# sczhou/CodeFormer

Measured on NVIDIA H100. Metric: faces_per_sec_512x512_batch32, higher is better.
Workload: dtype f32 (split-fp16 operands on tensor cores, fp32 accumulate)

## Files before the change

### codeformer_b200/csrc/conv_tc.cu

```cuda

#include <cuda.h>
#include <cuda_fp16.h>
#include <cuda_runtime.h>
#include <stdint.h>

#include <stdlib.h>

#include <atomic>
#include <mutex>

#include "conv_tc.cuh"

namespace cfb {

__global__ void tc_absmax_kernel(const float* __restrict__ w, int64_t total, unsigned* __restrict__ slot) {
  float m = 0.f;
  for (int64_t i = (int64_t)blockIdx.x * blockDim.x + threadIdx.x; i < total; i += (int64_t)gridDim.x * blockDim.x)
    m = fmaxf(m, fabsf(w[i]));
#pragma unroll
  for (int o = 16; o > 0; o >>= 1) m = fmaxf(m, __shfl_xor_sync(0xffffffffu, m, o));
  if ((threadIdx.x & 31) == 0) atomicMax(slot, __float_as_uint(m));
}

__global__ void tc_split_weights_kernel(const float* __restrict__ w, __half* __restrict__ hi, __half* __restrict__ lo,
// ... 445 lines not shown
  int a_split;
  const float* in_scale;
  const float* in_shift;
  int in_act;
  const float* bias;
  const float* residual;
  int out_act;
  const float* sft_dec;
  const float* sft_scale;
  union {
    float sft_w;
    float prelu;
  };
  const float* wscale_inv;
  float* out;
  __half* pl_hi;
  __half* pl_lo;
  float* gn_part;
  int gn_cpg;
  const float* sft_wv;
#if CFB_TC_STAMPS
  long long* dbg;
#endif
};
#if CFB_TC_STAMPS
#define TC_STAMP(i) do { if (p.dbg != nullptr && blockIdx.x == 0) p.dbg[i] = clock64(); } while (0)
#else
#define TC_STAMP(i) do { } while (0)
#endif

constexpr int XF_SKEW = 128;
constexpr int TC_A_BYTES = 128 * 128;

template <int BN>
struct TcCfg {
  static_assert(BN == 64 || BN == 128, "the wgmma engine runs 64- or 128-wide n-tiles");
  static constexpr bool WIDE = BN == 128;
  static constexpr int MMA_WARPS = WIDE ? 8 : 4;
  static constexpr int EPI_WARPS = WIDE ? 4 : 8;
  static constexpr int THREADS = WIDE ? 512 : 32 * (MMA_WARPS + 1 + EPI_WARPS);
  static constexpr int B_BYTES = BN * 128;
  static constexpr int STAGE_BYTES = 2 * TC_A_BYTES + 2 * B_BYTES;
  static constexpr int STAGES = 3;
  static constexpr int SLOT_PITCH = BN + 4;
  static constexpr int SLOT_BYTES = 128 * SLOT_PITCH * 4;
  static constexpr int SLOTS = 1;
  static constexpr int STG_BYTES = WIDE ? 0 : 8 * 4096;
  static constexpr int TAIL_BYTES = SLOT_BYTES + 1024  + 512  + STG_BYTES;
  static constexpr int SMEM_BYTES = STAGES * STAGE_BYTES + TAIL_BYTES;
  static constexpr int H_A_PLANE = 23 * 1024;
  static constexpr int H_A_SLOT = 2 * H_A_PLANE;
  static constexpr int H_A_SLOTS = 2;
  static constexpr int H_B_SLOT = 2 * B_BYTES;
  static constexpr int H_B_SLOTS = WIDE ? 2 : 4;
  static constexpr int H_SMEM_BYTES = H_A_SLOTS * H_A_SLOT + H_B_SLOTS * H_B_SLOT + TAIL_BYTES;
  static constexpr int XF_WARPS = WIDE ? 2 : 4;
  static constexpr int XF_THREADS = 32 * (MMA_WARPS + 1 + EPI_WARPS + XF_WARPS + 1);
  static_assert(!WIDE || XF_THREADS == THREADS, "the 128-wide transform variant fills the pad warps exactly");
  static constexpr int X_A_SLOTS = 2;
  static constexpr int X_A_PLANE2 = H_A_PLANE + XF_SKEW;
  static constexpr int X_B_SLOTS = H_B_SLOTS;
  static constexpr int X_SMEM_BYTES = X_A_SLOTS * H_A_SLOT + X_B_SLOTS * H_B_SLOT + TAIL_BYTES;
};

template <int BN, int CPG, bool HALO, bool XF, bool GEN = false, bool K1 = false, bool CM = false, bool SILU = false,
          bool P1 = false, bool PRELU = false>
__global__ void __launch_bounds__(XF ? TcCfg<BN>::XF_THREADS : TcCfg<BN>::THREADS, 1)
conv_tc_kernel(const __grid_constant__ CUtensorMap tmA_hi, const __grid_constant__ CUtensorMap tmA_lo,
               const __grid_constant__ CUtensorMap tmB_hi, const __grid_constant__ CUtensorMap tmB_lo, const TcParams p) {
  static_assert(!XF || HALO, "the fused operand transform exists for the halo engine only");
  static_assert(!GEN || (XF && CPG == 0), "the generalised addressing exists for the fused-transform engine only");
  static_assert(!PRELU || (BN == 64 && CPG == 0 && !K1 && !CM && !SILU && !P1 && (GEN || !HALO)),
                "the PReLU epilogue is built for the generalised and the per-tap engines");
  static_assert(!K1 || (XF && !GEN && CPG == 0), "K1 = fused transform of a 1x1 conv (patch = tile): its own instantiation");
  using Cfg = TcCfg<BN>;
  constexpr bool WIDE = Cfg::WIDE;
  static_assert(!WIDE || (HALO && !GEN && !K1 && CPG != 2), "128-wide tiles exist for the 3x3 / Upsample halo engine");
  static_assert(!CM || (BN == 64 && HALO && !GEN && !K1), "channel-major tiles exist for the 64-channel 3x3 / Upsample halo convs");
  static_assert(!P1 || (!SILU && !K1 && (GEN || WIDE || CM || !HALO)),
                "the single-pass fp16 variant is built for the generalised, 128-wide, channel-major and per-tap engines");
  constexpr int MMA_WARPS = Cfg::MMA_WARPS, EPI_WARPS = Cfg::EPI_WARPS;
  constexpr int A_SLOTS = XF ? Cfg::X_A_SLOTS : Cfg::H_A_SLOTS;
  constexpr int STAGES = Cfg::STAGES;
  constexpr int STAGE_BYTES = Cfg::STAGE_BYTES;
  const int first_tile = (int)blockIdx.x;
  const int tile_step = (int)gridDim.x;
  extern __shared__ uint8_t smem_raw[];
  uint8_t* smem = reinterpret_cast<uint8_t*>((reinterpret_cast<uintptr_t>(smem_raw) + 1023) & ~(uintptr_t)1023);
  constexpr int NRING = HALO ? (XF ? Cfg::X_B_SLOTS : Cfg::H_B_SLOTS) : STAGES;
  constexpr int RING_BYTES = HALO ? Cfg::H_B_SLOT : STAGE_BYTES;
  uint8_t* ring_base = HALO ? smem + A_SLOTS * Cfg::H_A_SLOT : smem;
  float* acc_slot = reinterpret_cast<float*>(ring_base + NRING * RING_BYTES);
  uint64_t* bars = reinterpret_cast<uint64_t*>(ring_base + NRING * RING_BYTES + Cfg::SLOT_BYTES);
  uint64_t* full = bars;
  uint64_t* empty = bars + NRING;
  uint64_t* cfull = bars + 2 * NRING;
  uint64_t* cempty = bars + 2 * NRING + Cfg::SLOTS;
  uint64_t* afull = bars + 2 * NRING + 2 * Cfg::SLOTS;
  uint64_t* aempty = afull + 3;
  uint64_t* araw = aempty + 3;
  uint8_t* stage_buf = reinterpret_cast<uint8_t*>(bars) + 512;

  constexpr int NWARPS = (XF ? Cfg::XF_THREADS : Cfg::THREADS) / 32;
  const int pwarp = __shfl_sync(0xffffffffu, (int)(threadIdx.x >> 5), 0);
  const int ridx = NWARPS - 1 - pwarp;
  const int warp = pwarp < MMA_WARPS ? 1 : (ridx == 0 ? 0 : ridx + 1);
  const int lane = threadIdx.x & 31;
  bool aborted = false;
  if constexpr (WIDE) {
    if (pwarp >= MMA_WARPS) wg_regs_dec<96>();
  }
  if (threadIdx.x == 0) TC_STAMP(0);

  if (warp == 0 && lane == 0) {
    for (int a = 0; a < 3; ++a) {
      mbar_init(smem_u32(afull + a), XF ? Cfg::XF_WARPS : 1);
      mbar_init(smem_u32(aempty + a), MMA_WARPS);
      mbar_init(smem_u32(araw + a), 1);
    }
    asm volatile("prefetch.tensormap [%0];" ::"l"(&tmA_hi) : "memory");
    asm volatile("prefetch.tensormap [%0];" ::"l"(&tmA_lo) : "memory");
    asm volatile("prefetch.tensormap [%0];" ::"l"(&tmB_hi) : "memory");
    asm volatile("prefetch.tensormap [%0];" ::"l"(&tmB_lo) : "memory");
    for (int s = 0; s < NRING; ++s) { mbar_init(smem_u32(full + s), 1); mbar_init(smem_u32(empty + s), MMA_WARPS); }
    for (int a = 0; a < Cfg::SLOTS; ++a) {
      mbar_init(smem_u32(cfull + a), MMA_WARPS);
      mbar_init(smem_u32(cempty + a), EPI_WARPS);
    }
    asm volatile("fence.mbarrier_init.release.cluster;" ::: "memory");
  }
  __syncthreads();
  pdl_launch_dependents();
  pdl_wait();
  if (threadIdx.x == 0) TC_STAMP(1);

  const int total_tiles = p.m_tiles * p.n_tiles;
  const int nk = p.taps * p.kblocks;

  if (warp == 0) {
    {
      int stage = 0;
      uint32_t phase = 0;
      int aslot = 0;
// ... 38 lines not shown
            }
          }
        } else {
          for (int tap = 0; tap < p.taps; ++tap) {
            int r, s, btap = tap;
            if (p.up4) { r = (tap >> 1) + par_y; s = (tap & 1) + par_x; btap = (mt & 3) * 4 + tap; }
            else { r = (p.taps == 9) ? tap / 3 : 0; s = (p.taps == 9) ? tap - r * 3 : 0; }
            for (int kb = 0; kb < p.kblocks; ++kb) {
              mbar_wait<500>(smem_u32(empty + stage), phase ^ 1, aborted); if (aborted) goto teardown;
              if (elect_one()) {
                if (tile == first_tile && tap == 0 && kb == 0) TC_STAMP(2);
                const uint32_t sa = smem_u32(smem + stage * STAGE_BYTES);
                const int hh = p.heads > 1 ? n % p.heads : 0, nimg = p.heads > 1 ? n / p.heads : n;
                const int a_img = p.a_img_per_head ? n : nimg;
                const int ac = p.a_c0 + hh * p.a_c_head + kb * 64, bc = p.b_c0 + hh * p.b_c_head + kb * 64;
                const int brow = nt * BN + hh * p.b_r_head;
                const int b3 = p.b_batched ? nimg : btap;
                const uint32_t fb = smem_u32(full + stage);
                const bool drop = p.fault && blockIdx.x == 0 && tile == first_tile && kb == 0 && tap == 0;
                mbar_expect_tx(fb, (uint32_t)(P1 ? TC_A_BYTES + Cfg::B_BYTES : Cfg::STAGE_BYTES));
                tma_load_4d(sa, &tmA_hi, fb, ac, x0 + s - p.pad, y0 + r - p.pad, a_img);
                if constexpr (!P1) tma_load_4d(sa + TC_A_BYTES, &tmA_lo, fb, ac, x0 + s - p.pad, y0 + r - p.pad, a_img);
                if (!drop) tma_load_3d(sa + 2 * TC_A_BYTES, &tmB_hi, fb, bc, brow, b3);
                if constexpr (!P1) tma_load_3d(sa + 2 * TC_A_BYTES + Cfg::B_BYTES, &tmB_lo, fb, bc, brow, b3);
              }
              __syncwarp();
              if (++stage == STAGES) { stage = 0; phase ^= 1; }
            }
          }
        }
      }
    }
  } else if (warp == 1) {
    if constexpr (WIDE) wg_regs_inc<160>();
    {
      constexpr bool N128 = WIDE || CM;
      constexpr int MH = N128 ? 1 : 2;
      const uint32_t a_sbo = HALO ? (uint32_t)(p.PW * 128) : 1024u;
      const uint32_t a_half = HALO ? (uint32_t)(8 * p.PW * 128) : 8192u;
      const int wq = (int)(threadIdx.x >> 5) & 3;
      const int wg = (int)(threadIdx.x >> 7);
      const uint32_t bar_id = 2u + (uint32_t)wg;
      const uint32_t slot_base = smem_u32(acc_slot);
      int stage = 0;
      uint32_t phase = 0;
      int slot = 0;
      uint32_t slot_phase = 0;
      int aslot = 0;
      uint32_t aphase = 0;
      float acc[MH][N128 ? 64 : 32];
      if constexpr (N128) {
        float run[64];
        auto hand_off = [&]() -> bool {
          mbar_wait(smem_u32(cempty + slot), slot_phase ^ 1, aborted);
          if (wg_any(aborted, bar_id)) return true;
          const int row = wg * 64 + wq * 16 + (lane >> 2);
          uint32_t e0;
          asm volatile("mov.b32 %0, %1;" : "=r"(e0)
                       : "r"(slot_base + (uint32_t)(slot * Cfg::SLOT_BYTES) + (uint32_t)((row * Cfg::SLOT_PITCH + 2 * (lane & 3)) * 4)));
#pragma unroll
          for (int j = 0; j < 16; ++j) {
#pragma unroll
            for (int h8 = 0; h8 < 2; ++h8) {
              const uint32_t e = e0 + (uint32_t)((8 * h8 * Cfg::SLOT_PITCH + 8 * j) * 4);
              asm volatile("st.shared.v2.f32 [%0], {%1, %2};" ::"r"(e), "f"(run[4 * j + 2 * h8]), "f"(run[4 * j + 2 * h8 + 1])
                           : "memory");
            }
          }
          __syncwarp();
          if (lane == 0) mbar_arrive(smem_u32(cfull + slot));
          if (++slot == Cfg::SLOTS) { slot = 0; slot_phase ^= 1; }
          return false;
        };
        for (int tile = first_tile; tile < total_tiles; tile += tile_step) {
          const int par = p.up4 ? ((tile / p.n_tiles) & 3) : 0;
          const int par_y = par >> 1, par_x = par & 1;
          for (int c0 = 0; c0 < nk; c0 += p.chunk) {
            const int c1 = min(c0 + p.chunk, nk);
            uint32_t prev_empty = 0, prev_aempty = 0;
            for (int it = c0; it < c1; ++it) {
              const int kb = it / p.taps;
              const int tap = it - kb * p.taps;
              if (tap == 0) {
                mbar_wait(smem_u32(afull + aslot), aphase, aborted);
                if (wg_any(aborted, bar_id)) { wg_wait_all(); aborted = true; goto teardown; }
              }
              int r = (p.taps == 9) ? tap / 3 : 0;
              int sft = (p.taps == 9) ? tap - r * 3 : 0;
              if (p.up4) { r = (tap >> 1) + par_y; sft = (tap & 1) + par_x; }
              const uint32_t a_hi0 = smem_u32(smem + aslot * Cfg::H_A_SLOT) + (uint32_t)((r * p.PW + sft) * 128) +
                                     (uint32_t)wg * a_half;
              const uint32_t a_lo0 = a_hi0 + (uint32_t)(XF ? Cfg::X_A_PLANE2 : Cfg::H_A_PLANE);
              const uint32_t bsm = smem_u32(ring_base + stage * RING_BYTES);
              mbar_wait(smem_u32(full + stage), phase, aborted);
              if (wg_any(aborted, bar_id)) { wg_wait_all(); aborted = true; goto teardown; }
              wg_fence();
#pragma unroll
              for (int k = 0; k < 4; ++k) {
                const uint64_t db_hi = wg_desc(bsm + 32 * k, 1024u), db_lo = wg_desc(bsm + Cfg::B_BYTES + 32 * k, 1024u);
                const uint64_t da_hi = wg_desc(a_hi0 + 32 * k, a_sbo), da_lo = wg_desc(a_lo0 + 32 * k, a_sbo);
                if constexpr (P1 && CM) {
                  wg_mma_64x128(acc[0], db_hi, da_hi, (it == c0 && k == 0) ? 0u : 1u);
                } else if constexpr (P1) {
                  wg_mma_64x128(acc[0], da_hi, db_hi, (it == c0 && k == 0) ? 0u : 1u);
                } else if constexpr (CM) {
                  wg_mma_64x128(acc[0], db_hi, da_lo, (it == c0 && k == 0) ? 0u : 1u);
                  wg_mma_64x128(acc[0], db_lo, da_hi, 1u);
                  wg_mma_64x128(acc[0], db_hi, da_hi, 1u);
                } else {
                  wg_mma_64x128(acc[0], da_lo, db_hi, (it == c0 && k == 0) ? 0u : 1u);
                  wg_mma_64x128(acc[0], da_hi, db_lo, 1u);
                  wg_mma_64x128(acc[0], da_hi, db_hi, 1u);
                }
              }
              wg_commit();
              if constexpr (WIDE) {
                if (it == 0 && tile != first_tile) {
                  if (hand_off()) { wg_wait_all(); aborted = true; goto teardown; }
                }
              }
              wg_wait_1();
              __syncwarp();
              mbar_arrive_if(prev_empty, lane == 0 && prev_empty != 0);
              mbar_arrive_if(prev_aempty, lane == 0 && prev_aempty != 0);
              prev_empty = smem_u32(empty + stage);
              prev_aempty = tap == p.taps - 1 ? smem_u32(aempty + aslot) : 0u;
              if (++stage == NRING) { stage = 0; phase ^= 1; }
              if (tap == p.taps - 1 && ++aslot == A_SLOTS) { aslot = 0; aphase ^= 1; }
            }
            wg_wait_all();
            __syncwarp();
            mbar_arrive_if(prev_empty, lane == 0);
            mbar_arrive_if(prev_aempty, lane == 0 && prev_aempty != 0);
            if constexpr (CM) {
              mbar_wait(smem_u32(cempty + slot), slot_phase ^ 1, aborted);
              if (wg_any(aborted, bar_id)) { aborted = true; goto teardown; }
              const uint32_t st0 = slot_base + (uint32_t)(slot * Cfg::SLOT_BYTES) +
                                   (uint32_t)((2 * (lane & 3) * Cfg::SLOT_PITCH + wq * 16 + (lane >> 2)) * 4);
#pragma unroll
              for (int j = 0; j < 16; ++j) {
#pragma unroll
                for (int h8 = 0; h8 < 2; ++h8) {
#pragma unroll
                  for (int e = 0; e < 2; ++e) {
                    const uint32_t a = st0 + (uint32_t)(((8 * j + e) * Cfg::SLOT_PITCH + 8 * h8) * 4);
                    asm volatile("st.shared.f32 [%0], %1;" ::"r"(a), "f"(acc[0][4 * j + 2 * h8 + e]) : "memory");
                  }
                }
              }
              __syncwarp();
              if (lane == 0) mbar_arrive(smem_u32(cfull + slot));
              if (++slot == Cfg::SLOTS) { slot = 0; slot_phase ^= 1; }
              continue;
            }
            if constexpr (WIDE) {
#pragma unroll
              for (int i = 0; i < 64; ++i) run[i] = __fadd_rn(c0 == 0 ? 0.f : run[i], acc[0][i]);
            }
          }
        }
        if constexpr (WIDE) {
          if (first_tile < total_tiles && hand_off()) { aborted = true; goto teardown; }
        }
      } else {
      for (int tile = first_tile; tile < total_tiles; tile += tile_step) {
        const int par = p.up4 ? ((tile / p.n_tiles) & 3) : 0;
        const int par_y = par >> 1, par_x = par & 1;
        for (int it = 0; it < nk; ++it) {
          uint32_t a_hi0, a_lo0, bsm;
          int tap = 0;
          if constexpr (HALO) {
            const int kb = it / p.taps;
            tap = it - kb * p.taps;
            if (tap == 0) { mbar_wait(smem_u32(afull + aslot), aphase, aborted); if (wg_any(aborted)) { aborted = true; goto teardown; } }
            int r = (p.taps == 9) ? tap / 3 : 0;
            int sft = (p.taps == 9) ? tap - r * 3 : 0;
            if (p.up4) { r = (tap >> 1) + par_y; sft = (tap & 1) + par_x; }
            const uint32_t aoff = (uint32_t)((r * p.PW + sft) * 128);
            a_hi0 = smem_u32(smem + aslot * Cfg::H_A_SLOT) + aoff;
            a_lo0 = a_hi0 + (uint32_t)(XF ? Cfg::X_A_PLANE2 : Cfg::H_A_PLANE);
            bsm = smem_u32(ring_base + stage * RING_BYTES);
          } else {
            a_hi0 = smem_u32(smem + stage * STAGE_BYTES);
            a_lo0 = a_hi0 + TC_A_BYTES;
            bsm = a_hi0 + 2 * TC_A_BYTES;
          }
          mbar_wait(smem_u32(full + stage), phase, aborted); if (wg_any(aborted)) { aborted = true; goto teardown; }
          if (blockIdx.x == 0 && threadIdx.x == 0 && tile == first_tile && it == 0) TC_STAMP(3);
          const uint32_t first = (it % p.chunk) == 0 ? 1u : 0u;
          wg_fence();
#pragma unroll
          for (int k = 0; k < 4; ++k) {
            const uint64_t db_hi = wg_desc(bsm + 32 * k, 1024u), db_lo = wg_desc(bsm + Cfg::B_BYTES + 32 * k, 1024u);
#pragma unroll
            for (int mh = 0; mh < 2; ++mh) {
// ... 40 lines not shown
      }
      }
    }
  } else if (XF && warp == 2 + EPI_WARPS + Cfg::XF_WARPS) {
    if constexpr (XF) {
      int aslot = 0;
      uint32_t aphase = 0;
      for (int tile = first_tile; tile < total_tiles; tile += tile_step) {
        const int mt0 = tile / p.n_tiles;
        const int mt = p.up4 ? (mt0 >> 2) : mt0;
        const int per_img = p.tiles_x * p.tiles_y;
        const int n = mt / per_img;
        const int rem = mt - n * per_img;
        const int ty = rem / p.tiles_x, tx = rem - ty * p.tiles_x;
        const int y0 = ty * p.BH, x0 = tx * p.BW;
        for (int kb = 0; kb < p.kblocks; ++kb) {
          mbar_wait<500>(smem_u32(aempty + aslot), aphase ^ 1, aborted); if (aborted) goto teardown;
          if (elect_one()) {
            const uint32_t sa = smem_u32(smem + aslot * Cfg::H_A_SLOT);
            const uint32_t rb = smem_u32(araw + aslot);
            const bool src0 = kb < p.a_split;
            const CUtensorMap* src = src0 ? &tmA_hi : &tmA_lo;
            const int c0 = (src0 ? kb : kb - p.a_split) * 64;
            if (tile == first_tile && kb == 0) TC_STAMP(10);
            mbar_expect_tx(rb, (uint32_t)(2 * p.PW * p.PH * 128));
            tma_load_4d(sa, src, rb, c0, x0 - p.pad, y0 - p.pad, n);
            tma_load_4d(sa + Cfg::X_A_PLANE2, src, rb, c0 + 32, x0 - p.pad, y0 - p.pad, n);
          }
          __syncwarp();
          if (++aslot == A_SLOTS) { aslot = 0; aphase ^= 1; }
        }
      }
    }
  } else if ((XF || WIDE) && warp >= 2 + EPI_WARPS) {

    if constexpr (XF) {
      constexpr int XFW = Cfg::XF_WARPS;
      constexpr int RPP = 4 * XFW;
      constexpr int XF_PW = 10, XF_PH = 18, XF_ROWS = XF_PW * XF_PH;
      constexpr int NPASS = (XF_ROWS + RPP - 1) / RPP;
      constexpr int NPASS1 = (128 + RPP - 1) / RPP;
      const int t = (warp - (2 + EPI_WARPS)) * 32 + lane;
      const int j = t & 7, rsub = t >> 3;
      const int pl = j >> 2, c0 = 2 * (j & 3);
      const int mode = p.in_scale ? (p.in_act == IN_SILU ? 2 : 1) : 0;
      const int Hin = GEN ? p.Hin : p.tiles_y * p.BH, Win = GEN ? p.Win : p.tiles_x * p.BW;
      const int Cin = p.kblocks * 64;
      float amax = 0.f;
      int aslot = 0;
      uint32_t aphase = 0;
      for (int tile = first_tile; tile < total_tiles; tile += tile_step) {
        const int mt0 = tile / p.n_tiles;
        const int mt = p.up4 ? (mt0 >> 2) : mt0;
        const int per_img = p.tiles_x * p.tiles_y;
        const int n = mt / per_img;
        const int rem = mt - n * per_img;
        const int ty = rem / p.tiles_x, tx = rem - ty * p.tiles_x;
        const int y0 = ty * p.BH - p.pad, x0 = tx * p.BW - p.pad;
        const bool border = !K1 && (y0 < 0 || x0 < 0 || y0 + XF_PH > Hin || x0 + XF_PW > Win);
        for (int kb = 0; kb < p.kblocks; ++kb) {
          float sc[8], sh[8];
          if (mode) {
            const int nn = GEN ? min(n, p.N - 1) : n;
            const float* sp = p.in_scale + (int64_t)nn * Cin + kb * 64 + j * 8;
            const float* hp = p.in_shift + (int64_t)nn * Cin + kb * 64 + j * 8;
            const float4 s0 = __ldg(reinterpret_cast<const float4*>(sp)), s1 = __ldg(reinterpret_cast<const float4*>(sp + 4));
            const float4 h0 = __ldg(reinterpret_cast<const float4*>(hp)), h1 = __ldg(reinterpret_cast<const float4*>(hp + 4));
// ... 72 lines not shown
    int slot = 0;
    uint32_t slot_phase = 0;
    float omax = 0.f;
    for (int tile = first_tile; tile < total_tiles; tile += tile_step) {
      const int pm = tile / p.n_tiles, nt = tile - pm * p.n_tiles;
      const int mt = pm;
      const int mtl = p.up4 ? (mt >> 2) : mt;
      const int per_img = p.tiles_x * p.tiles_y;
      const int nb = mtl / per_img;
      const int rem = mtl - nb * per_img;
      const bool hsplit = !HALO && p.heads > 1 && !p.out_per_head;
      const int n = hsplit ? nb / p.heads : nb;
      const int ty = rem / p.tiles_x, tx = rem - ty * p.tiles_x;
      const int h = bw_shift >= 0 ? (row >> bw_shift) : row / BW, w = row - h * BW;
      int oy = ty * BH + h, ox = tx * BW + w;
      if (p.up4) { oy = 2 * oy + ((mt & 3) >> 1); ox = 2 * ox + (mt & 1); }
      const int64_t pix = ((int64_t)n * p.Ho + oy) * p.Wo + ox;
      const int64_t off_tile = (((int64_t)n * p.Ho + (p.up4 ? 2 * ty * BH + ((mt & 3) >> 1) : ty * BH)) * p.Wo +
                                (p.up4 ? 2 * tx * BW + (mt & 1) : tx * BW)) * (HALO ? p.Cout : p.out_pitch);
      const int col0 = nt * BN + cbase + (hsplit ? (nb % p.heads) * p.o_c_head : 0);
      const int64_t off0 = pix * (HALO ? p.Cout : p.out_pitch) + col0;
      const bool row_in = whole_tiles || (oy < p.Ho && ox < p.Wo);
      if (!GEN && p.residual && row_in) {
#pragma unroll
        for (int j = 0; j < HC; j += 32) asm volatile("prefetch.global.L2 [%0];" ::"l"(p.residual + off0 + j));
      }
      if (p.sft_dec && row_in) {
#pragma unroll
        for (int j = 0; j < HC; j += 32) {
          asm volatile("prefetch.global.L2 [%0];" ::"l"(p.sft_dec + off0 + j));
          asm volatile("prefetch.global.L2 [%0];" ::"l"(p.sft_scale + off0 + j));
        }
      }
      float acc[WIDE ? 1 : HC];
      if constexpr (WIDE) {
        mbar_wait<250>(smem_u32(cfull + slot), slot_phase, aborted); if (aborted) goto teardown;
      } else {
#pragma unroll
        for (int j = 0; j < HC; ++j) acc[j] = 0.f;
        for (int it0 = 0; it0 < nk; it0 += p.chunk) {
          mbar_wait<250>(smem_u32(cfull + slot), slot_phase, aborted); if (aborted) goto teardown;
          const uint32_t srow = smem_u32(acc_slot) + (uint32_t)(slot * Cfg::SLOT_BYTES) + (uint32_t)((row * Cfg::SLOT_PITCH + cbase) * 4);
#pragma unroll
          for (int c0 = 0; c0 < HC; c0 += 4) {
            const float4 v = lds128f(srow + (uint32_t)(c0 * 4));
            acc[c0] += v.x; acc[c0 + 1] += v.y; acc[c0 + 2] += v.z; acc[c0 + 3] += v.w;
          }
          asm volatile("" ::: "memory");
          __syncwarp();
          if (lane == 0) mbar_arrive(smem_u32(cempty + slot));
          if (++slot == Cfg::SLOTS) { slot = 0; slot_phase ^= 1; }
        }
      }
      if (warp == 2 && lane == 0 && tile == first_tile) TC_STAMP(7);
      if (warp == 2 && lane == 0 && tile == first_tile + tile_step) TC_STAMP(17);
      const uint32_t stg = smem_u32(stage_buf) + (uint32_t)(warp - 2) * 4096u;
      const uint32_t stg_w = stg + (uint32_t)lane * 128u;
      const int cch = lane & 7, rsub = lane >> 3;
      if constexpr (GEN) {
        const int Hs = p.sub ? (p.Ho >> 1) : p.Ho, Ws = p.sub ? (p.Wo >> 1) : p.Wo;
#pragma unroll
        for (int q = 0; q < HC; q += 32) {
#pragma unroll
          for (int j = 0; j < 8; ++j)
            sts128f(stg_w + (uint32_t)((j ^ (lane & 7)) << 4), acc[q + 4 * j] * wsi, acc[q + 4 * j + 1] * wsi, acc[q + 4 * j + 2] * wsi,
                    acc[q + 4 * j + 3] * wsi);
          __syncwarp();
          const int colq = col0 + q + cch * 4;
// ... 15 lines not shown
#pragma unroll
          for (int it = 0; it < 8; ++it)
            rres[it] = (p.residual && pixs[it] >= 0) ? __ldg(reinterpret_cast<const float4*>(p.residual + pixs[it] * p.res_pitch + colq))
                                                     : make_float4(0.f, 0.f, 0.f, 0.f);
#pragma unroll
          for (int it = 0; it < 8; ++it) {
            const int r = it * 4 + rsub;
            float4 v = lds128f(stg + (uint32_t)(r * 128 + ((cch ^ (r & 7)) << 4)));
            v.x += bv.x + rres[it].x; v.y += bv.y + rres[it].y; v.z += bv.z + rres[it].z; v.w += bv.w + rres[it].w;
            if constexpr (PRELU) {
              v.x = v.x > 0.f ? v.x : p.prelu * v.x; v.y = v.y > 0.f ? v.y : p.prelu * v.y;
              v.z = v.z > 0.f ? v.z : p.prelu * v.z; v.w = v.w > 0.f ? v.w : p.prelu * v.w;
            } else if (p.out_act == OUT_LRELU || p.out_act == OUT_RELU) {
              const float sl = p.out_act == OUT_LRELU ? 0.2f : 0.f;
              v.x = v.x > 0.f ? v.x : sl * v.x; v.y = v.y > 0.f ? v.y : sl * v.y;
              v.z = v.z > 0.f ? v.z : sl * v.z; v.w = v.w > 0.f ? v.w : sl * v.w;
            } else if (SILU) {
              v.x = tc_silu_out(v.x); v.y = tc_silu_out(v.y); v.z = tc_silu_out(v.z); v.w = tc_silu_out(v.w);
            }
            if (pixs[it] >= 0) {
              if (p.residual2) {
                const float4 r2 = __ldg(reinterpret_cast<const float4*>(p.residual2 + pixs[it] * p.res2_pitch + colq));
                v.x = fmaf(v.x, p.post_scale, r2.x); v.y = fmaf(v.y, p.post_scale, r2.y);
                v.z = fmaf(v.z, p.post_scale, r2.z); v.w = fmaf(v.w, p.post_scale, r2.w);
              }
              *reinterpret_cast<float4*>(p.out + pixs[it] * p.out_pitch + p.out_c0 + colq) = v;
            }
          }
          __syncwarp();
        }
      } else {
      const uint32_t slot_q = smem_u32(acc_slot) + (uint32_t)(slot * Cfg::SLOT_BYTES) +
                              (uint32_t)(((lg * 32 + rsub) * Cfg::SLOT_PITCH + cbase + cch * 4) * 4);
#pragma unroll
      for (int q = 0; q < HC; q += 32) {
        if constexpr (!WIDE) {
#pragma unroll
          for (int j = 0; j < 8; ++j)
            sts128f(stg_w + (uint32_t)((j ^ (lane & 7)) << 4), acc[q + 4 * j] * wsi, acc[q + 4 * j + 1] * wsi, acc[q + 4 * j + 2] * wsi,
                    acc[q + 4 * j + 3] * wsi);
          __syncwarp();
        }
        const int colq = col0 + q + cch * 4;
        float4 bv = make_float4(0.f, 0.f, 0.f, 0.f);
        if (p.bias) bv = __ldg(reinterpret_cast<const float4*>(p.bias + colq));
        constexpr int RB = (XF || WIDE) ? 4 : 8;
        float s0 = 0.f, q0 = 0.f, s1 = 0.f, q1 = 0.f, k0 = 0.f, k1 = 0.f;
#pragma unroll
        for (int ib = 0; ib < 8; ib += RB) {
        int64_t offs[RB];
        bool inside[RB];
#pragma unroll
        for (int k = 0; k < RB; ++k) {
          const int it = ib + k;
          const int trow = lg * 32 + it * 4 + rsub;
          const int hh = bw_shift >= 0 ? (trow >> bw_shift) : trow / BW, ww = trow - hh * BW;
          offs[k] = off_tile + colq + hh * SH + ww * SW;
          inside[k] = whole_tiles || ((ty * BH + hh) * ts < p.Ho && (tx * BW + ww) * ts < p.Wo);
        }
        float4 rres[RB];
#pragma unroll
        for (int k = 0; k < RB; ++k)
          rres[k] = (p.residual && inside[k]) ? __ldg(reinterpret_cast<const float4*>(p.residual + offs[k])) : make_float4(0.f, 0.f, 0.f, 0.f);
#pragma unroll
        for (int k = 0; k < RB; ++k) {
          const int it = ib + k;
          const int r = it * 4 + rsub;
          float4 v;
          if constexpr (WIDE) {
            v = lds128f(slot_q + (uint32_t)((it * 4 * Cfg::SLOT_PITCH + q) * 4));
            v.x = __fmul_rn(v.x, wsi); v.y = __fmul_rn(v.y, wsi); v.z = __fmul_rn(v.z, wsi); v.w = __fmul_rn(v.w, wsi);
          } else {
            v = lds128f(stg + (uint32_t)(r * 128 + ((cch ^ (r & 7)) << 4)));
          }
          const int64_t off = offs[k];
          v.x += bv.x + rres[k].x; v.y += bv.y + rres[k].y; v.z += bv.z + rres[k].z; v.w += bv.w + rres[k].w;
          if constexpr (PRELU) {
            v.x = v.x > 0.f ? v.x : p.prelu * v.x; v.y = v.y > 0.f ? v.y : p.prelu * v.y;
            v.z = v.z > 0.f ? v.z : p.prelu * v.z; v.w = v.w > 0.f ? v.w : p.prelu * v.w;
          } else if (p.out_act == OUT_LRELU) {
            v.x = v.x > 0.f ? v.x : 0.2f * v.x; v.y = v.y > 0.f ? v.y : 0.2f * v.y;
            v.z = v.z > 0.f ? v.z : 0.2f * v.z; v.w = v.w > 0.f ? v.w : 0.2f * v.w;
          } else if (p.out_act == OUT_GELU) {
            v.x = 0.5f * v.x * (1.f + erff(v.x * 0.70710678118654752440f));
            v.y = 0.5f * v.y * (1.f + erff(v.y * 0.70710678118654752440f));
            v.z = 0.5f * v.z * (1.f + erff(v.z * 0.70710678118654752440f));
            v.w = 0.5f * v.w * (1.f + erff(v.w * 0.70710678118654752440f));
          } else if (p.out_act == OUT_RELU) {
            v.x = fmaxf(v.x, 0.f); v.y = fmaxf(v.y, 0.f); v.z = fmaxf(v.z, 0.f); v.w = fmaxf(v.w, 0.f);
          } else if (SILU) {
            v.x = tc_silu_out(v.x); v.y = tc_silu_out(v.y); v.z = tc_silu_out(v.z); v.w = tc_silu_out(v.w);
          }
          if (p.sft_dec && inside[k]) {
            const float4 d = __ldg(reinterpret_cast<const float4*>(p.sft_dec + off));
            const float4 sc = __ldg(reinterpret_cast<const float4*>(p.sft_scale + off));
            float sw = p.sft_w;
            if constexpr (!XF) { if (p.sft_wv) { const float t = __ldg(p.sft_wv + n); sw = t > 0.f ? t : 0.f; } }
            v.x = d.x + sw * (d.x * sc.x + v.x); v.y = d.y + sw * (d.y * sc.y + v.y);
            v.z = d.z + sw * (d.z * sc.z + v.z); v.w = d.w + sw * (d.w * sc.w + v.w);
          }
          if (!inside[k]) v = make_float4(0.f, 0.f, 0.f, 0.f);
          if (p.out && inside[k]) *reinterpret_cast<float4*>(p.out + off) = v;
// ... 12 lines not shown
            if (it == 0) { k0 = v.x; k1 = v.z; }
            const float a = v.x - k0, b = v.y - k0, c = v.z - k1, d = v.w - k1;
            s0 += a + b; q0 += fmaf(a, a, b * b);
            s1 += c + d; q1 += fmaf(c, c, d * d);
          } else if constexpr (CPG >= 4) {
            if (it == 0) k0 = v.x;
            const float a = v.x - k0, b = v.y - k0, c = v.z - k0, d = v.w - k0;
            s0 += (a + b) + (c + d);
            q0 += fmaf(a, a, b * b) + fmaf(c, c, d * d);
          }
        }
        }
        if constexpr (CPG > 0) {
          constexpr float NL = CPG == 2 ? 16.f : 32.f;
          gn_lane_moments(s0, q0, k0, NL);
          if constexpr (CPG == 2) gn_lane_moments(s1, q1, k1, NL);
          gn_merge_xor(s0, q0, 8, NL); gn_merge_xor(s0, q0, 16, 2.f * NL);
          if constexpr (CPG == 2) { gn_merge_xor(s1, q1, 8, NL); gn_merge_xor(s1, q1, 16, 2.f * NL); }
          if constexpr (CPG >= 8) gn_merge_xor(s0, q0, 1, 4.f * NL);
          if constexpr (CPG >= 16) gn_merge_xor(s0, q0, 2, 8.f * NL);
          constexpr int CL = (CPG >= 4) ? CPG / 4 : 1;
          if (rsub == 0 && (cch & (CL - 1)) == 0) {
            float* gp = p.gn_part + ((int64_t)mt * 4 + lg) * 64;
            if constexpr (CPG == 2) {
              *reinterpret_cast<float4*>(gp + (colq / 2) * 2) = make_float4(s0, q0, s1, q1);
            } else {
              *reinterpret_cast<float2*>(gp + (colq / CPG) * 2) = make_float2(s0, q0);
            }
          }
        }
        __syncwarp();
      }
      }
      if constexpr (WIDE) {
        if (lane == 0) mbar_arrive(smem_u32(cempty + slot));
        if (++slot == Cfg::SLOTS) { slot = 0; slot_phase ^= 1; }
      }
      if (warp == 2 && lane == 0 && tile == first_tile) TC_STAMP(16);
      if (warp == 2 && lane == 0 && tile == first_tile + tile_step) TC_STAMP(18);
    }
    if (omax > 65504.f) report_overflow();
    if (warp == 2 && lane == 0) TC_STAMP(13);
  }

teardown:
  if (aborted) {
    const long long t0 = clock64();
    while (clock64() - t0 < 400000) {}
  }
  __syncthreads();
  if (threadIdx.x == 0) TC_STAMP(8);
}

int tc_bind_status_word(unsigned* host_mapped_dev_ptr, long long wait_limit_cycles) {
  const unsigned zero = 0;
  CFB_CUDA(cudaMemcpyToSymbol(g_status_host, &host_mapped_dev_ptr, sizeof(host_mapped_dev_ptr)));
  CFB_CUDA(cudaMemcpyToSymbol(g_wait_limit, &wait_limit_cycles, sizeof(wait_limit_cycles)));
  CFB_CUDA(cudaMemcpyToSymbol(g_abort, &zero, sizeof(zero)));
  return 0;
}
static std::atomic<int> g_inject_fault{0};
static std::atomic<long long*> g_stamps{nullptr};
int tc_set_stamps(long long* dev_ptr) { g_stamps.store(dev_ptr); return 0; }
int tc_inject_fault(int kind) { g_inject_fault.store(kind); return 0; }
int tc_clear_abort() {
  const unsigned zero = 0;
  CFB_CUDA(cudaMemcpyToSymbol(g_abort, &zero, sizeof(zero)));
// ... 79 lines not shown
  if (a.mode == CONV_UP && a.ksize != 3) return false;
  if (128 % BW != 0) return false;
  if ((int64_t)a.N * (a.Ho / BH + 1) * (a.Wo / BW + 1) * (a.Cout / 64) > 0x7fffffffLL) return false;
  return true;
}

bool tc_tiles_exact(const ConvArgs& a) {
  if (!tc_supported(a)) return false;
  const TcGeom g = tc_geometry(a);
  const int Wt = a.mode == CONV_UP ? a.W : a.Wo, Ht = a.mode == CONV_UP ? a.H : a.Ho;
  return Wt % g.BW == 0 && Ht % g.BH == 0;
}

bool tc_can_xform(const ConvArgs& a) {
  static const int mode = [] { const char* e = getenv("CFB_TC_XFORM"); return e ? atoi(e) : 1; }();
  if (a.gen) return tc_supported(a);
  if (mode == 0 || !tc_supported(a) || a.mode != CONV_SAME || !(a.ksize == 3 || (a.ksize == 1 && a.halo1x1 && a.Cout % 128 == 0))) return false;
  if (mode == 3 && !(a.Cout % 128 == 0 && a.Cin >= 128 && (int64_t)a.Ho * a.Wo >= 4096)) return false;
  return tc_geometry(a).halo;
}

size_t tc_scratch_bytes(const ConvArgs& a) {
  if (!tc_supported(a)) return 0;
  const int Hp = a.mode == CONV_SAME ? a.Ho : a.H, Wp = a.mode == CONV_SAME ? a.Wo : a.W;
  const size_t plane = ((size_t)a.N * Hp * Wp * a.Cin * 2 + 1023) / 1024 * 1024;
  return 2 * plane;
}

struct TcMaps { CUtensorMap a_hi, a_lo, b_hi, b_lo; };

template <int BN, int CPG, bool HALO, bool XF = false, bool GEN = false, bool K1 = false, bool CM = false, bool SILU = false,
          bool P1 = false, bool PRELU = false>
static int launch_tc2(const TcMaps& m, const TcParams& p, int sm_count, cudaStream_t st) {
  using Cfg = TcCfg<BN>;
  constexpr int SMEM = XF ? Cfg::X_SMEM_BYTES : (HALO ? Cfg::H_SMEM_BYTES : Cfg::SMEM_BYTES);
  constexpr int THREADS = XF ? Cfg::XF_THREADS : Cfg::THREADS;
  static_assert(SMEM <= 232448, "shared memory budget");
  static std::atomic<uint64_t> attr_done{0};
  int dev = 0;
  CFB_CUDA(cudaGetDevice(&dev));
  const uint64_t bit = 1ull << (dev & 63);
  if (!(attr_done.load(std::memory_order_acquire) & bit)) {
    CFB_CUDA(cudaFuncSetAttribute(conv_tc_kernel<BN, CPG, HALO, XF, GEN, K1, CM, SILU, P1, PRELU>, cudaFuncAttributeMaxDynamicSharedMemorySize, SMEM));
    attr_done.fetch_or(bit, std::memory_order_release);
  }
  const int total = p.m_tiles * p.n_tiles;
  const int grid = total < sm_count ? total : sm_count;
  CFB_LAUNCH_PDL((conv_tc_kernel<BN, CPG, HALO, XF, GEN, K1, CM, SILU, P1, PRELU>), dim3((unsigned)grid), dim3(THREADS), (size_t)SMEM, st,
                 m.a_hi, m.a_lo, m.b_hi, m.b_lo, p);
  return 0;
}
template <int CPG>
static int launch_tc_p1(const TcMaps& m, const TcParams& p, int sm_count, cudaStream_t st, bool gen, int tile) {
  constexpr bool T = true, F = false;
  const bool halo3 = p.PW == 10 && p.PH == 18;
  if (p.out_act != OUT_SILU) {
    if (gen) {
      if constexpr (CPG == 0) {
        if (p.xform && halo3) return launch_tc2<64, 0, T, T, T, F, F, F, T>(m, p, sm_count, st);
      }
    } else if (tile == 128 && halo3) {
      if constexpr (CPG == 4 || CPG == 8 || CPG == 16) {
        if (p.xform) return launch_tc2<128, CPG, T, T, F, F, F, F, T>(m, p, sm_count, st);
      }
      if constexpr (CPG != 2) {
        if (!p.xform) return launch_tc2<128, CPG, T, F, F, F, F, F, T>(m, p, sm_count, st);
      }
// ... 643 lines not shown
```

Measured before the change: 189.8.

## Give channel-major convs a one-pass 512-thread config with double-buffered accumulators

Adds a ONCE configuration for channel-major 64-wide non-P1 tiles. It uses 512 threads with setmaxnreg register rebalancing, MMA warps placed in the high warpgroup, and the full-K accumulator handed off once per tile instead of staging. When the K loop fits in one chunk, the MMA warps ping-pong between two 64-float accumulator sets, so the previous tile's store to shared memory overlaps the next tile's first wgmma. This raises register pressure in the MMA warps, drops the staging buffer, and changes the epilogue's work split.

```diff
diff --git a/codeformer_b200/csrc/conv_tc.cu b/codeformer_b200/csrc/conv_tc.cu
--- a/codeformer_b200/csrc/conv_tc.cu
+++ b/codeformer_b200/csrc/conv_tc.cu
@@ -501,20 +501,25 @@
 constexpr int XF_SKEW = 128;
 constexpr int TC_A_BYTES = 128 * 128;
 
-template <int BN>
+template <int BN, bool CM1 = false>
 struct TcCfg {
   static_assert(BN == 64 || BN == 128, "the wgmma engine runs 64- or 128-wide n-tiles");
+  static_assert(!CM1 || BN == 64, "channel-major tiles are 64 channels wide");
   static constexpr bool WIDE = BN == 128;
+  static constexpr bool ONCE = WIDE || CM1;
   static constexpr int MMA_WARPS = WIDE ? 8 : 4;
-  static constexpr int EPI_WARPS = WIDE ? 4 : 8;
-  static constexpr int THREADS = WIDE ? 512 : 32 * (MMA_WARPS + 1 + EPI_WARPS);
+  static constexpr int EPI_WARPS = ONCE ? 4 : 8;
+  static constexpr int THREADS = ONCE ? 512 : 32 * (MMA_WARPS + 1 + EPI_WARPS);
+  static constexpr int MMA_REGS = WIDE ? 160 : 176;
+  static constexpr int OTHER_REGS = WIDE ? 96 : 112;
+  static_assert(!ONCE || 32 * MMA_WARPS * MMA_REGS + (THREADS - 32 * MMA_WARPS) * OTHER_REGS == 65536, "register split");
   static constexpr int B_BYTES = BN * 128;
   static constexpr int STAGE_BYTES = 2 * TC_A_BYTES + 2 * B_BYTES;
   static constexpr int STAGES = 3;
   static constexpr int SLOT_PITCH = BN + 4;
   static constexpr int SLOT_BYTES = 128 * SLOT_PITCH * 4;
   static constexpr int SLOTS = 1;
-  static constexpr int STG_BYTES = WIDE ? 0 : 8 * 4096;
+  static constexpr int STG_BYTES = ONCE ? 0 : 8 * 4096;
   static constexpr int TAIL_BYTES = SLOT_BYTES + 1024  + 512  + STG_BYTES;
   static constexpr int SMEM_BYTES = STAGES * STAGE_BYTES + TAIL_BYTES;
   static constexpr int H_A_PLANE = 23 * 1024;
@@ -524,8 +529,9 @@
   static constexpr int H_B_SLOTS = WIDE ? 2 : 4;
   static constexpr int H_SMEM_BYTES = H_A_SLOTS * H_A_SLOT + H_B_SLOTS * H_B_SLOT + TAIL_BYTES;
   static constexpr int XF_WARPS = WIDE ? 2 : 4;
-  static constexpr int XF_THREADS = 32 * (MMA_WARPS + 1 + EPI_WARPS + XF_WARPS + 1);
-  static_assert(!WIDE || XF_THREADS == THREADS, "the 128-wide transform variant fills the pad warps exactly");
+  static constexpr int XF_ROLE_WARPS = MMA_WARPS + 1 + EPI_WARPS + XF_WARPS + 1;
+  static constexpr int XF_THREADS = ONCE ? THREADS : 32 * XF_ROLE_WARPS;
+  static_assert(!ONCE || 32 * XF_ROLE_WARPS <= THREADS, "the transform variants of ONCE fit the whole warpgroups");
   static constexpr int X_A_SLOTS = 2;
   static constexpr int X_A_PLANE2 = H_A_PLANE + XF_SKEW;
   static constexpr int X_B_SLOTS = H_B_SLOTS;
@@ -534,7 +540,7 @@
 
 template <int BN, int CPG, bool HALO, bool XF, bool GEN = false, bool K1 = false, bool CM = false, bool SILU = false,
           bool P1 = false, bool PRELU = false>
-__global__ void __launch_bounds__(XF ? TcCfg<BN>::XF_THREADS : TcCfg<BN>::THREADS, 1)
+__global__ void __launch_bounds__(XF ? TcCfg<BN, CM && !P1>::XF_THREADS : TcCfg<BN, CM && !P1>::THREADS, 1)
 conv_tc_kernel(const __grid_constant__ CUtensorMap tmA_hi, const __grid_constant__ CUtensorMap tmA_lo,
                const __grid_constant__ CUtensorMap tmB_hi, const __grid_constant__ CUtensorMap tmB_lo, const TcParams p) {
   static_assert(!XF || HALO, "the fused operand transform exists for the halo engine only");
@@ -542,8 +548,8 @@
   static_assert(!PRELU || (BN == 64 && CPG == 0 && !K1 && !CM && !SILU && !P1 && (GEN || !HALO)),
                 "the PReLU epilogue is built for the generalised and the per-tap engines");
   static_assert(!K1 || (XF && !GEN && CPG == 0), "K1 = fused transform of a 1x1 conv (patch = tile): its own instantiation");
-  using Cfg = TcCfg<BN>;
-  constexpr bool WIDE = Cfg::WIDE;
+  using Cfg = TcCfg<BN, CM && !P1>;
+  constexpr bool WIDE = Cfg::WIDE, ONCE = Cfg::ONCE;
   static_assert(!WIDE || (HALO && !GEN && !K1 && CPG != 2), "128-wide tiles exist for the 3x3 / Upsample halo engine");
   static_assert(!CM || (BN == 64 && HALO && !GEN && !K1), "channel-major tiles exist for the 64-channel 3x3 / Upsample halo convs");
   static_assert(!P1 || (!SILU && !K1 && (GEN || WIDE || CM || !HALO)),
@@ -571,13 +577,15 @@
   uint8_t* stage_buf = reinterpret_cast<uint8_t*>(bars) + 512;
 
   constexpr int NWARPS = (XF ? Cfg::XF_THREADS : Cfg::THREADS) / 32;
+  constexpr bool MMA_HIGH = ONCE && !WIDE;
   const int pwarp = __shfl_sync(0xffffffffu, (int)(threadIdx.x >> 5), 0);
-  const int ridx = NWARPS - 1 - pwarp;
-  const int warp = pwarp < MMA_WARPS ? 1 : (ridx == 0 ? 0 : ridx + 1);
+  const bool mma_warp = MMA_HIGH ? pwarp >= NWARPS - MMA_WARPS : pwarp < MMA_WARPS;
+  const int ridx = (MMA_HIGH ? NWARPS - MMA_WARPS : NWARPS) - 1 - pwarp;
+  const int warp = mma_warp ? 1 : (ridx == 0 ? 0 : ridx + 1);
   const int lane = threadIdx.x & 31;
   bool aborted = false;
-  if constexpr (WIDE) {
-    if (pwarp >= MMA_WARPS) wg_regs_dec<96>();
+  if constexpr (ONCE) {
+    if (!mma_warp) wg_regs_dec<Cfg::OTHER_REGS>();
   }
   if (threadIdx.x == 0) TC_STAMP(0);
 
@@ -682,14 +690,14 @@
       }
     }
   } else if (warp == 1) {
-    if constexpr (WIDE) wg_regs_inc<160>();
+    if constexpr (ONCE) wg_regs_inc<Cfg::MMA_REGS>();
     {
       constexpr bool N128 = WIDE || CM;
       constexpr int MH = N128 ? 1 : 2;
       const uint32_t a_sbo = HALO ? (uint32_t)(p.PW * 128) : 1024u;
       const uint32_t a_half = HALO ? (uint32_t)(8 * p.PW * 128) : 8192u;
       const int wq = (int)(threadIdx.x >> 5) & 3;
-      const int wg = (int)(threadIdx.x >> 7);
+      const int wg = MMA_HIGH ? 0 : (int)(threadIdx.x >> 7);
       const uint32_t bar_id = 2u + (uint32_t)wg;
       const uint32_t slot_base = smem_u32(acc_slot);
       int stage = 0;
@@ -701,20 +709,40 @@
       float acc[MH][N128 ? 64 : 32];
       if constexpr (N128) {
         float run[64];
-        auto hand_off = [&]() -> bool {
+        auto hand_off = [&](const float (&v)[64]) -> bool {
           mbar_wait(smem_u32(cempty + slot), slot_phase ^ 1, aborted);
           if (wg_any(aborted, bar_id)) return true;
-          const int row = wg * 64 + wq * 16 + (lane >> 2);
-          uint32_t e0;
-          asm volatile("mov.b32 %0, %1;" : "=r"(e0)
-                       : "r"(slot_base + (uint32_t)(slot * Cfg::SLOT_BYTES) + (uint32_t)((row * Cfg::SLOT_PITCH + 2 * (lane & 3)) * 4)));
-#pragma unroll
-          for (int j = 0; j < 16; ++j) {
-#pragma unroll
-            for (int h8 = 0; h8 < 2; ++h8) {
-              const uint32_t e = e0 + (uint32_t)((8 * h8 * Cfg::SLOT_PITCH + 8 * j) * 4);
-              asm volatile("st.shared.v2.f32 [%0], {%1, %2};" ::"r"(e), "f"(run[4 * j + 2 * h8]), "f"(run[4 * j + 2 * h8 + 1])
-                           : "memory");
+          if constexpr (CM) {
+            uint32_t e0;
+            asm volatile("mov.b32 %0, %1;" : "=r"(e0)
+                         : "r"(slot_base + (uint32_t)(slot * Cfg::SLOT_BYTES) +
+                               (uint32_t)((2 * (lane & 3) * Cfg::SLOT_PITCH + wq * 16 + (lane >> 2)) * 4)));
+#pragma unroll
+            for (int j = 0; j < 16; ++j) {
+#pragma unroll
+              for (int h8 = 0; h8 < 2; ++h8) {
+#pragma unroll
+                for (int e = 0; e < 2; ++e) {
+                  float x = v[4 * j + 2 * h8 + e];
+                  asm volatile("" : "+f"(x));
+                  const uint32_t a = e0 + (uint32_t)(((8 * j + e) * Cfg::SLOT_PITCH + 8 * h8) * 4);
+                  asm volatile("st.shared.f32 [%0], %1;" ::"r"(a), "f"(__fadd_rn(0.f, x)) : "memory");
+                }
+              }
+            }
+          } else {
+            const int row = wg * 64 + wq * 16 + (lane >> 2);
+            uint32_t e0;
+            asm volatile("mov.b32 %0, %1;" : "=r"(e0)
+                         : "r"(slot_base + (uint32_t)(slot * Cfg::SLOT_BYTES) + (uint32_t)((row * Cfg::SLOT_PITCH + 2 * (lane & 3)) * 4)));
+#pragma unroll
+            for (int j = 0; j < 16; ++j) {
+#pragma unroll
+              for (int h8 = 0; h8 < 2; ++h8) {
+                const uint32_t e = e0 + (uint32_t)((8 * h8 * Cfg::SLOT_PITCH + 8 * j) * 4);
+                asm volatile("st.shared.v2.f32 [%0], {%1, %2};" ::"r"(e), "f"(v[4 * j + 2 * h8]), "f"(v[4 * j + 2 * h8 + 1])
+                             : "memory");
+              }
             }
           }
           __syncwarp();
@@ -722,6 +750,76 @@
           if (++slot == Cfg::SLOTS) { slot = 0; slot_phase ^= 1; }
           return false;
         };
+        if (CM && ONCE && nk <= p.chunk) {
+          float acc1[64];
+          uint32_t prev_empty = 0, prev_aempty = 0;
+          auto kblock = [&](float (&d)[64], int it, int par) -> bool {
+            const int kb = it / p.taps;
+            const int tap = it - kb * p.taps;
+            if (tap == 0) {
+              mbar_wait(smem_u32(afull + aslot), aphase, aborted);
+              if (wg_any(aborted, bar_id)) return true;
+            }
+            int r = (p.taps == 9) ? tap / 3 : 0;
+            int sft = (p.taps == 9) ? tap - r * 3 : 0;
+            if (p.up4) { r = (tap >> 1) + (par >> 1); sft = (tap & 1) + (par & 1); }
+            const uint32_t a_hi0 = smem_u32(smem + aslot * Cfg::H_A_SLOT) + (uint32_t)((r * p.PW + sft) * 128);
+            const uint32_t bsm = smem_u32(ring_base + stage * RING_BYTES);
+            const uint32_t a_lo0 = a_hi0 + (uint32_t)(XF ? Cfg::X_A_PLANE2 : Cfg::H_A_PLANE);
+            mbar_wait(smem_u32(full + stage), phase, aborted);
+            if (wg_any(aborted, bar_id)) return true;
+            wg_fence();
+#pragma unroll
+            for (int k = 0; k < 4; ++k) {
+              const uint64_t db_hi = wg_desc(bsm + 32 * k, 1024u), db_lo = wg_desc(bsm + Cfg::B_BYTES + 32 * k, 1024u);
+              const uint64_t da_hi = wg_desc(a_hi0 + 32 * k, a_sbo), da_lo = wg_desc(a_lo0 + 32 * k, a_sbo);
+              if constexpr (P1) {
+                wg_mma_64x128(d, db_hi, da_hi, (it == 0 && k == 0) ? 0u : 1u);
+              } else {
+                wg_mma_64x128(d, db_hi, da_lo, (it == 0 && k == 0) ? 0u : 1u);
+                wg_mma_64x128(d, db_lo, da_hi, 1u);
+                wg_mma_64x128(d, db_hi, da_hi, 1u);
+              }
+            }
+            wg_commit();
+            wg_wait_1();
+            __syncwarp();
+            mbar_arrive_if(prev_empty, lane == 0 && prev_empty != 0);
+            mbar_arrive_if(prev_aempty, lane == 0 && prev_aempty != 0);
+            prev_empty = smem_u32(empty + stage);
+            prev_aempty = tap == p.taps - 1 ? smem_u32(aempty + aslot) : 0u;
+            if (++stage == NRING) { stage = 0; phase ^= 1; }
+            if (tap == p.taps - 1 && ++aslot == A_SLOTS) { aslot = 0; aphase ^= 1; }
+            return false;
+          };
+          auto tile_mma = [&](float (&cur)[64], const float (&prev)[64], int tile) -> bool {
+            const int par = p.up4 ? ((tile / p.n_tiles) & 3) : 0;
+            for (int it = 0; it < nk; ++it) {
+              if (kblock(cur, it, par)) return true;
+              if (it == 0 && tile != first_tile && hand_off(prev)) return true;
+            }
+            return false;
+          };
+          auto last_tile = [&](const float (&v)[64]) -> bool {
+            wg_wait_all();
+            __syncwarp();
+            mbar_arrive_if(prev_empty, lane == 0);
+            mbar_arrive_if(prev_aempty, lane == 0 && prev_aempty != 0);
+            return hand_off(v);
+          };
+          for (int tile = first_tile;; tile += 2 * tile_step) {
+            if (tile_mma(acc[0], acc1, tile)) { wg_wait_all(); aborted = true; goto teardown; }
+            if (tile + tile_step >= total_tiles) {
+              if (last_tile(acc[0])) { aborted = true; goto teardown; }
+              break;
+            }
+            if (tile_mma(acc1, acc[0], tile + tile_step)) { wg_wait_all(); aborted = true; goto teardown; }
+            if (tile + 2 * tile_step >= total_tiles) {
+              if (last_tile(acc1)) { aborted = true; goto teardown; }
+              break;
+            }
+          }
+        } else {
         for (int tile = first_tile; tile < total_tiles; tile += tile_step) {
           const int par = p.up4 ? ((tile / p.n_tiles) & 3) : 0;
           const int par_y = par >> 1, par_x = par & 1;
@@ -764,9 +862,9 @@
                 }
               }
               wg_commit();
-              if constexpr (WIDE) {
+              if constexpr (ONCE) {
                 if (it == 0 && tile != first_tile) {
-                  if (hand_off()) { wg_wait_all(); aborted = true; goto teardown; }
+                  if (hand_off(run)) { wg_wait_all(); aborted = true; goto teardown; }
                 }
               }
               wg_wait_1();
@@ -782,7 +880,7 @@
             __syncwarp();
             mbar_arrive_if(prev_empty, lane == 0);
             mbar_arrive_if(prev_aempty, lane == 0 && prev_aempty != 0);
-            if constexpr (CM) {
+            if constexpr (!ONCE) {
               mbar_wait(smem_u32(cempty + slot), slot_phase ^ 1, aborted);
               if (wg_any(aborted, bar_id)) { aborted = true; goto teardown; }
               const uint32_t st0 = slot_base + (uint32_t)(slot * Cfg::SLOT_BYTES) +
@@ -801,16 +899,15 @@
               __syncwarp();
               if (lane == 0) mbar_arrive(smem_u32(cfull + slot));
               if (++slot == Cfg::SLOTS) { slot = 0; slot_phase ^= 1; }
-              continue;
-            }
-            if constexpr (WIDE) {
+            } else {
 #pragma unroll
               for (int i = 0; i < 64; ++i) run[i] = __fadd_rn(c0 == 0 ? 0.f : run[i], acc[0][i]);
             }
           }
         }
-        if constexpr (WIDE) {
-          if (first_tile < total_tiles && hand_off()) { aborted = true; goto teardown; }
+        if constexpr (ONCE) {
+          if (first_tile < total_tiles && hand_off(run)) { aborted = true; goto teardown; }
+        }
         }
       } else {
       for (int tile = first_tile; tile < total_tiles; tile += tile_step) {
@@ -917,7 +1014,8 @@
         }
       }
     }
-  } else if ((XF || WIDE) && warp >= 2 + EPI_WARPS) {
+  } else if (XF && Cfg::XF_ROLE_WARPS < NWARPS && warp > 2 + EPI_WARPS + Cfg::XF_WARPS) {
+  } else if ((XF || ONCE) && warp >= 2 + EPI_WARPS) {
 
     if constexpr (XF) {
       constexpr int XFW = Cfg::XF_WARPS;
@@ -1056,8 +1154,8 @@
           asm volatile("prefetch.global.L2 [%0];" ::"l"(p.sft_scale + off0 + j));
         }
       }
-      float acc[WIDE ? 1 : HC];
-      if constexpr (WIDE) {
+      float acc[ONCE ? 1 : HC];
+      if constexpr (ONCE) {
         mbar_wait<250>(smem_u32(cfull + slot), slot_phase, aborted); if (aborted) goto teardown;
       } else {
 #pragma unroll
@@ -1139,9 +1237,9 @@
       } else {
       const uint32_t slot_q = smem_u32(acc_slot) + (uint32_t)(slot * Cfg::SLOT_BYTES) +
                               (uint32_t)(((lg * 32 + rsub) * Cfg::SLOT_PITCH + cbase + cch * 4) * 4);
-#pragma unroll
+#pragma unroll (CM ? 1 : HC / 32)
       for (int q = 0; q < HC; q += 32) {
-        if constexpr (!WIDE) {
+        if constexpr (!ONCE) {
 #pragma unroll
           for (int j = 0; j < 8; ++j)
             sts128f(stg_w + (uint32_t)((j ^ (lane & 7)) << 4), acc[q + 4 * j] * wsi, acc[q + 4 * j + 1] * wsi, acc[q + 4 * j + 2] * wsi,
@@ -1151,7 +1249,7 @@
         const int colq = col0 + q + cch * 4;
         float4 bv = make_float4(0.f, 0.f, 0.f, 0.f);
         if (p.bias) bv = __ldg(reinterpret_cast<const float4*>(p.bias + colq));
-        constexpr int RB = (XF || WIDE) ? 4 : 8;
+        constexpr int RB = (XF || ONCE) ? 4 : 8;
         float s0 = 0.f, q0 = 0.f, s1 = 0.f, q1 = 0.f, k0 = 0.f, k1 = 0.f;
 #pragma unroll
         for (int ib = 0; ib < 8; ib += RB) {
@@ -1174,7 +1272,7 @@
           const int it = ib + k;
           const int r = it * 4 + rsub;
           float4 v;
-          if constexpr (WIDE) {
+          if constexpr (ONCE) {
             v = lds128f(slot_q + (uint32_t)((it * 4 * Cfg::SLOT_PITCH + q) * 4));
             v.x = __fmul_rn(v.x, wsi); v.y = __fmul_rn(v.y, wsi); v.z = __fmul_rn(v.z, wsi); v.w = __fmul_rn(v.w, wsi);
           } else {
@@ -1253,7 +1351,7 @@
         __syncwarp();
       }
       }
-      if constexpr (WIDE) {
+      if constexpr (ONCE) {
         if (lane == 0) mbar_arrive(smem_u32(cempty + slot));
         if (++slot == Cfg::SLOTS) { slot = 0; slot_phase ^= 1; }
       }
@@ -1399,7 +1497,7 @@
 template <int BN, int CPG, bool HALO, bool XF = false, bool GEN = false, bool K1 = false, bool CM = false, bool SILU = false,
           bool P1 = false, bool PRELU = false>
 static int launch_tc2(const TcMaps& m, const TcParams& p, int sm_count, cudaStream_t st) {
-  using Cfg = TcCfg<BN>;
+  using Cfg = TcCfg<BN, CM && !P1>;
   constexpr int SMEM = XF ? Cfg::X_SMEM_BYTES : (HALO ? Cfg::H_SMEM_BYTES : Cfg::SMEM_BYTES);
   constexpr int THREADS = XF ? Cfg::XF_THREADS : Cfg::THREADS;
   static_assert(SMEM <= 232448, "shared memory budget");
```

New measurement: 194.9 (median of 6 runs). 2.7% higher.
